# dist1ll/pomcpp

Hardware: AMD Instinct MI355X
Metric: env_steps_per_sec (higher is better)
Workload: dtype int32

## Files before the change

pomcpp_amd/csrc/pom_copy.h:

```cpp
#ifndef POM_COPY_H_
#define POM_COPY_H_

#include <hip/hip_runtime.h>

#include <cstdint>

#include "pom_batch.h"
#include "pom_kernels.h"
#include "pom_packed.h"

struct CopyParams {
    const int64_t* src;
    int64_t first, count, n, n_pad;
    int64_t tile0;
    int32_t flags;
    uint32_t* state;
    uint32_t* snap;
    uint32_t* agent_mem;
    uint32_t* episode;
    uint32_t* terminal;
    uint32_t* out_state;
    uint32_t* out_agent_mem;
    uint32_t* out_episode;
    uint32_t* out_terminal;
// ... 29 lines not shown
        } else {
            const uint32_t* st = p.state + (s >> 4) * POM_TILE_DWORDS;
            for (int k = lane; k < POM_COL_ITEMS; k += 64) pom_col_copy_item(tile, ec, st, (int)(s & 15), k);
        }
        if (p.agent_mem && lane < 8) {
            const int64_t half = (int64_t)(lane >> 2) * 4 * p.n_pad, a = lane & 3;
            p.out_agent_mem[half + e * 4 + a] = from_snap ? 0u : p.agent_mem[half + s * 4 + a];
        }
        if (!from_snap) {
            if (lane == 0) p.out_episode[e] = p.episode[s];
            if (p.terminal)
                for (int k = lane; k < POM_REC_DWORDS; k += 64) p.out_terminal[e * POM_REC_DWORDS + k] = p.terminal[s * POM_REC_DWORDS + k];
        }
    }
    __syncthreads();
    store_tile16_x4(p.out_state + t * POM_TILE_DWORDS, POM_TILE_ENVS, tile, lane);
}

template <bool SCATTER>
__global__ __launch_bounds__(64) void pom_copy_scatter_kernel(CopyParams p)
{
    const int lane = threadIdx.x;
    const int64_t t = p.tile0 + blockIdx.x;
    const bool from_snap = (p.flags & POM_COPY_FROM_SNAPSHOT) != 0;
    if (SCATTER) {
        const uint4* g = reinterpret_cast<const uint4*>(p.out_state + t * POM_TILE_DWORDS);
        uint4* d = reinterpret_cast<uint4*>(p.state + t * POM_TILE_DWORDS);
#pragma unroll
        for (int k = lane; k < POM_TILE_DWORDS / 4; k += 64) d[k] = g[k];
    }
    for (int ec = 0; ec < POM_TILE_ENVS; ec++) {
// ... 22 lines not shown
```

pomcpp_amd/csrc/pom_kernels.h:

```cpp
#ifndef POM_KERNELS_H_
#define POM_KERNELS_H_

#include <hip/hip_ext.h>
#include <hip/hip_runtime.h>

#include <climits>
#include <cstdint>

#include "pom_batch.h"
#include "pom_boardgen_body.h"
#include "pom_packed.h"
#include "pom_policy_body.h"
#include "pom_step_body.h"

enum {
    ROW_BOARD = POM_REC_BOARD,
    ROW_BOMBS = POM_REC_BOMBS,
    ROW_FLAMES = POM_REC_FLAMES,
    ROW_BDEST = POM_REC_DWORDS,
    ROW_STACK = POM_REC_DWORDS + 5,
    ROW_CLAIMS = POM_REC_DWORDS + 5,
    LDS_ROWS = POM_REC_DWORDS + 36
};
static_assert(POM_REC_DWORDS % 2 == 0, "the one-lane shapes move the record in groups of 1 or 2 rows");
// ... 63 lines not shown
#pragma unroll
        for (int k = 0; k < (31 + G - 1) / G; k++)
            if (G * k + G - 1 < 31 || sub() + G * k < 31) cm[sub() + G * k] = 0u;
    }
    __device__ void claim(int c)
    {
        __hip_atomic_fetch_add(reinterpret_cast<uint32_t*>(claim_map() + (c & ~3)), 1u << (8 * (c & 3)), __ATOMIC_RELAXED, __HIP_MEMORY_SCOPE_WORKGROUP);
    }
    __device__ int claims(int c) const { return claim_map()[c]; }
    __device__ void set_cell(int c, int v) { if (owner()) put_cell(c, v); }
    __device__ void set_bomb(int s, int v) { if (owner()) put_bomb(s, v); }
    __device__ void set_flame(int s, int v) { if (owner()) put_flame(s, v); }
    __device__ void set_bdest(int i, int v) { if (owner()) put_bdest(i, v); }
    __device__ void set_frame(int d, int v) { if (owner()) t[(ROW_STACK + d) * EPW] = (uint32_t)v; }
};

struct StepParams {
    uint32_t* state;
    const uint32_t* snap;
    const int32_t* moves;
    int64_t* wave_counters;
    int64_t n, n_pad, env_offset;
    uint64_t seed;
    uint32_t tick0;
    const uint32_t* tick_base;
    int32_t dist, ticks, mode, auto_reset, max_steps;
    int64_t block0, block_end;
    uint32_t* terminal;
    uint32_t* agent_mem;
    uint32_t* episode;
// ... 84 lines not shown
    }
}
template <int EPW>
__device__ __forceinline__ void store_tile(uint32_t* col, int64_t np, const uint32_t* tile, int sub, int el)
{
    constexpr int GR = 64 / EPW;
    uint32_t* g = col + (int64_t)sub * np;
    const int64_t stride = (int64_t)GR * np;
    const uint32_t* l = tile + sub * EPW + el;
#pragma unroll 8
    for (int r0 = 0; r0 < POM_REC_DWORDS; r0 += GR) {
        *g = l[r0 * EPW];
        g += stride;
    }
}
template <int ROWS = POM_REC_DWORDS, int AUX = 0>
__device__ __forceinline__ void load_tile16_x4(const uint32_t* base, int64_t np, uint32_t* tile, int lane)
{
    static_assert(ROWS <= POM_REC_DWORDS, "inside the record");
    const uint32_t* g = base + (int64_t)(lane >> 2) * np + 4 * (lane & 3);
    const int64_t stride = 16 * np;
#pragma unroll
    for (int r0 = 0; r0 + 16 <= ROWS; r0 += 16) {
        __builtin_amdgcn_global_load_lds((const __attribute__((address_space(1))) void*)g,
                                         (__attribute__((address_space(3))) void*)(tile + r0 * 16), 16, 0, AUX);
        g += stride;
    }
    if (ROWS % 16 != 0 && (lane >> 2) < ROWS % 16)
        __builtin_amdgcn_global_load_lds((const __attribute__((address_space(1))) void*)g,
                                         (__attribute__((address_space(3))) void*)(tile + (ROWS / 16) * 16 * 16), 16, 0, AUX);
}
template <bool NT = false>
__device__ __forceinline__ void store_tile16_x4(uint32_t* base, int64_t np, const uint32_t* tile, int lane)
{
    constexpr int ROWS = POM_REC_DWORDS;
    uint4* g = reinterpret_cast<uint4*>(base + (int64_t)(lane >> 2) * np + 4 * (lane & 3));
    const int64_t stride = 4 * np;
    const uint4* l = reinterpret_cast<const uint4*>(tile) + lane;
    typedef uint32_t pom_u32x4 __attribute__((ext_vector_type(4)));
#pragma unroll
    for (int r0 = 0; r0 + 16 <= ROWS; r0 += 16) {
        if (NT) {
            const uint4 v = l[r0 * 4];
            __builtin_nontemporal_store(pom_u32x4{v.x, v.y, v.z, v.w}, reinterpret_cast<pom_u32x4*>(g));
        } else *g = l[r0 * 4];
        g += stride;
    }
    if (ROWS % 16 != 0 && (lane >> 2) < ROWS % 16) {
        if (NT) {
            const uint4 v = l[(ROWS / 16) * 16 * 4];
            __builtin_nontemporal_store(pom_u32x4{v.x, v.y, v.z, v.w}, reinterpret_cast<pom_u32x4*>(g));
        } else *g = l[(ROWS / 16) * 16 * 4];
    }
}
template <int EPW, int ROWS = POM_REC_DWORDS>
__device__ __forceinline__ void restart_column(uint32_t* tile, int el, const uint32_t* src, int lane)
{
    const uint32_t v0 = src[lane];
    const uint32_t v1 = lane + 64 < ROWS ? src[lane + 64] : 0u;
    if (lane < POM_REC_BOARD_DWORDS) {
        uint8_t* cells = reinterpret_cast<uint8_t*>(tile);
#pragma unroll
        for (int j = 0; j < 4; j++) cells[tile_cell_byte<EPW>(el, 4 * lane + j)] = (uint8_t)(v0 >> (8 * j));
    } else tile[lane * EPW + el] = v0;
    if (lane + 64 < ROWS) tile[(lane + 64) * EPW + el] = v1;
}
template <int EPW>
__device__ __forceinline__ void column_to_record(const uint32_t* tile, int el, uint32_t* dst, int lane)
{
    if (lane < POM_REC_BOARD_DWORDS) {
        const uint8_t* cells = reinterpret_cast<const uint8_t*>(tile);
        uint32_t v = 0;
#pragma unroll
        for (int j = 0; j < 4; j++) v |= (uint32_t)cells[tile_cell_byte<EPW>(el, 4 * lane + j)] << (8 * j);
        dst[lane] = v;
    } else dst[lane] = tile[lane * EPW + el];
    if (lane + 64 < POM_REC_DWORDS) dst[lane + 64] = tile[(lane + 64) * EPW + el];
}

__device__ __forceinline__ void lane_from_tile(PomLane& L, int& time_step, uint32_t& status, const uint32_t* t, int epw)
// ... 562 lines not shown
__device__ __forceinline__ uint32_t pom_chain_xcd()
{
    uint32_t x;
    asm volatile("s_getreg_b32 %0, hwreg(HW_REG_XCC_ID)" : "=s"(x));
    return x & 0xFu;
}
__device__ __forceinline__ bool pom_chain_enter(unsigned long long* word, uint32_t chain_xcd, uint32_t chain_seq0, uint32_t tape_len, uint64_t wait_limit,
                                                uint32_t* err, int lane, PomChainVisit& v)
{
    const uint32_t xcd = chain_xcd + 1u;
#if defined(POM_CHAIN_DIAG)
    v.t0 = (long long)__builtin_readcyclecounter();
    v.rt0 = (long long)wall_clock64();
#endif
    unsigned long long w = 0;
    if (lane == 0) w = __hip_atomic_fetch_add(word, 1ull << POM_CHAIN_TICKET_SHIFT, __ATOMIC_RELAXED, __HIP_MEMORY_SCOPE_AGENT);
    w = ((unsigned long long)(uint32_t)__builtin_amdgcn_readfirstlane((int)(w >> 32)) << 32) | (uint32_t)__builtin_amdgcn_readfirstlane((int)(uint32_t)w);
    const uint32_t visit = (uint32_t)(w >> POM_CHAIN_TICKET_SHIFT);
    v.dist = (int32_t)pom_chain_visit_distance(visit, chain_seq0);
#if defined(POM_CHAIN_DIAG)
    v.t1 = (long long)__builtin_readcyclecounter();
#endif
    int polls = 0;
    bool timed_out = false;
    if (!((uint32_t)w & POM_CHAIN_POISON) && (int32_t)pom_chain_visit_distance((uint32_t)w & POM_CHAIN_COUNT_MASK, visit) < 0) {
        const uint64_t t_wait0 = wall_clock64();
        for (;;) {
            __builtin_amdgcn_s_sleep(1);
            w = __hip_atomic_load(word, __ATOMIC_RELAXED, __HIP_MEMORY_SCOPE_AGENT);
            w = ((unsigned long long)(uint32_t)__builtin_amdgcn_readfirstlane((int)(w >> 32)) << 32) | (uint32_t)__builtin_amdgcn_readfirstlane((int)(uint32_t)w);
            polls++;
            if (((uint32_t)w & POM_CHAIN_POISON) || (int32_t)pom_chain_visit_distance((uint32_t)w & POM_CHAIN_COUNT_MASK, visit) >= 0) break;
            if (wall_clock64() - t_wait0 >= wait_limit) {
                timed_out = true;
                break;
            }
        }
    }
    (void)polls;
    const uint32_t was_on = (uint32_t)(w >> 32) & 0xFu;
    const bool poisoned = ((uint32_t)w & POM_CHAIN_POISON) != 0;
    const bool wrong_xcd = was_on != 0u && was_on != xcd;
    const bool off_tape = tape_len != 0u && (uint32_t)v.dist >= tape_len;
    if (poisoned || timed_out || wrong_xcd || off_tape) {
        if (lane == 0 && !poisoned) {
            __hip_atomic_fetch_or(word, (unsigned long long)POM_CHAIN_POISON, __ATOMIC_RELAXED, __HIP_MEMORY_SCOPE_AGENT);
            __hip_atomic_fetch_or(err, (uint32_t)(timed_out ? POM_CHAIN_E_TIMEOUT : wrong_xcd ? POM_CHAIN_E_XCD : POM_CHAIN_E_TAPE), __ATOMIC_RELAXED,
                                  __HIP_MEMORY_SCOPE_AGENT);
        }
        return false;
    }
#if defined(POM_CHAIN_DIAG)
    v.t2 = (long long)__builtin_readcyclecounter();
    v.polls = polls;
    v.visit = visit;
#endif
    v.done = 1ull + ((unsigned long long)(xcd - was_on) << 32);
    return true;
}
__device__ __forceinline__ void pom_chain_leave(unsigned long long* word, int lane, const PomChainVisit& v)
{
    asm volatile("s_waitcnt vmcnt(0)" ::: "memory");
    if (lane == 0) __hip_atomic_fetch_add(word, v.done, __ATOMIC_RELAXED, __HIP_MEMORY_SCOPE_AGENT);
}

__device__ __forceinline__ int64_t pom_xcd_tile_order(int64_t b, int64_t nb)
{
    const int64_t q = nb / 8, r = nb % 8, x = b % 8;
    return (x < r ? x * (q + 1) : r * (q + 1) + (x - r) * q) + b / 8;
}

template <bool CHAIN>
__device__ __forceinline__ uint32_t pom_load_shared(const uint32_t* ptr)
{
    return CHAIN ? __hip_atomic_load(ptr, __ATOMIC_RELAXED, __HIP_MEMORY_SCOPE_AGENT) : *ptr;
}

template <int EPW, int G, bool FRESH, bool POLICY = false, bool ATEND = false, bool SINGLE = false, bool CHAIN = false, bool OBS = false>
// ... 6 lines not shown
    static_assert(!POLICY || G == 4, "the policy runs one agent per lane of the quad");
    static_assert(!ATEND || G == 4, "the end-of-tick reset is built for the quad shape only");
    constexpr int OBS_ROWS = (obs_stage_vecs(OBS_PASS_ENVS_FUSED) * 16 + EPW * 4 - 1) / (EPW * 4);
    constexpr int OVERLAY = POLICY ? 44 : OBS ? OBS_ROWS : 0;
    constexpr int ROWS = POM_REC_DWORDS + OVERLAY > LDS_ROWS ? POM_REC_DWORDS + OVERLAY : LDS_ROWS;
    static_assert(ROWS >= LDS_ROWS, "the tick's scratch rows fit under the overlay");
    __shared__ __attribute__((aligned(16))) uint32_t tiles_[POM_WPB][ROWS * EPW];
    uint32_t* const tile = tiles_[POM_WPB == 1 ? 0 : threadIdx.x >> 6];
    uint8_t* const danger = reinterpret_cast<uint8_t*>(tile + POM_REC_DWORDS * EPW);
    uint32_t* const sets = tile + (POM_REC_DWORDS + 32) * EPW;
    const int lane = threadIdx.x & 63;
    int64_t tile_local;
    uint32_t chain_xcd = 0;
    if (CHAIN) {
        chain_xcd = pom_chain_xcd();
        const int64_t q = gridDim.x / 8;
        int64_t k_in_xcd = (int64_t)(blockIdx.x / 8) + p.chain_rot;
        if (k_in_xcd >= q) k_in_xcd -= q;
        tile_local = (int64_t)chain_xcd * q + k_in_xcd;
        if (chain_xcd >= 8u) {
            if (lane == 0) __hip_atomic_fetch_or(p.chain_err, (uint32_t)POM_CHAIN_E_XCD, __ATOMIC_RELAXED, __HIP_MEMORY_SCOPE_AGENT);
            return;
        }
        if (POM_WPB == 1 && p.block0 + tile_local >= p.block_end) return;
    } else {
#if defined(POM_NO_XCD_REMAP)
    tile_local = blockIdx.x;
#else
    {
        const int64_t b = blockIdx.x, nb = gridDim.x, q = nb / 8, r = nb % 8, x = b % 8;
        tile_local = (x < r ? x * (q + 1) : r * (q + 1) + (x - r) * q) + b / 8;
    }
#endif
    }
    if (POM_WPB > 1) {
        tile_local = tile_local * POM_WPB + (threadIdx.x >> 6);
        if (p.block0 + tile_local >= p.block_end) return;
    }
    const int64_t tile_id = p.block0 + tile_local;
    const int64_t np = p.n_pad;
    const bool env_mode = p.mode == POM_MODE_ENV;
    const int el = lane % EPW, sub = lane / EPW;
    const int64_t e_d = tile_id * EPW + el;
    uint32_t* col_d = p.state + pom_rec_col(e_d);
    const int ec = G == 1 ? el : lane >> 2;
    const int member = G == 1 ? 0 : lane & 3;
    const int64_t e = tile_id * EPW + ec;
    const bool owner = G == 1 ? sub == 0 : member == 0;
    const bool runs = G == 1 ? sub == 0 : true;
    const bool valid = runs && e < p.n;
    const uint32_t env_key = (uint32_t)(p.env_offset + e);
    uint32_t* t = tile + ec;

#if defined(POM_DIAG)
    const long long t_begin = (long long)clock64();
#endif
    long long c_steps = 0, c_episodes = 0, c_resets = 0, c_ub = 0;

    uint32_t tick0 = CHAIN ? p.tick0 : p.tick0 + *p.tick_base;
    PomChainVisit cv;
    if (CHAIN) {
        unsigned long long* const word = p.tile_seq + tile_id * POM_CHAIN_WORD_STRIDE;
        if (!pom_chain_enter(word, chain_xcd, p.chain_seq0, p.tape_len, p.chain_wait_limit, p.chain_err, lane, cv)) return;
        tick0 += (uint32_t)cv.dist;
        load_tile16_x4<POM_REC_DWORDS, 16>(p.state + tile_id * POM_TILE_DWORDS, POM_TILE_ENVS, tile, lane);
    } else if (EPW == 16) load_tile16_x4(p.state + tile_id * POM_TILE_DWORDS, POM_TILE_ENVS, tile, lane);
    else load_tile<EPW>(col_d, POM_TILE_ENVS, tile, sub);
    uint32_t m0 = 0, m1 = 0;
    if (POLICY) {
        m0 = pom_load_shared<CHAIN>(p.agent_mem + tile_id * 64 + lane);
        m1 = pom_load_shared<CHAIN>(p.agent_mem + 4 * np + tile_id * 64 + lane);
    }
    uint64_t draw0 = 0;
    int4 moves0 = make_int4(0, 0, 0, 0);
    constexpr bool TAKES_MOVES = SINGLE || G == 1;
    if (!POLICY) {
        if (TAKES_MOVES && p.moves) {
            if (valid) moves0 = reinterpret_cast<const int4*>(p.moves)[(CHAIN ? (int64_t)cv.dist * p.n : (int64_t)0) + e];
        } else {
            if (G == 4 && !SINGLE) {
            } else if (G == 4) draw0 = pom_rng_draw_half(p.seed, env_key, tick0, member >> 1);
            else draw0 = pom_rng_draw(p.seed, env_key, tick0);
        }
    }
    asm volatile("s_waitcnt vmcnt(0)" ::: "memory");
    PomLane L;
    int time_step = 0;
    uint32_t status = 0;
    lane_from_tile(L, time_step, status, t, EPW);
    bool restarted = false;

    LdsEnv<EPW, G> acc(tile, ec, member);
    PomStepper<LdsEnv<EPW, G>> stepper(acc, L);
#if defined(POM_TRUNC)
    L.trunc = p.trunc;
#endif
#if defined(POM_DIAG)
    for (int k = 0; k < POM_PH_N; k++) L.t_acc[k] = 0;
    L.t_last = t_begin;
    POM_STAMP(L, POM_PH_LOAD);
#endif

    const int n_ticks = SINGLE ? 1 : p.ticks;
    for (int tk = 0; tk < n_ticks; tk++) {
        if (ATEND) {
        } else if (FRESH) {
            const bool reload = valid && env_mode && p.auto_reset == POM_RESET_AT_START && (status & POM_ST_DONE);
            uint64_t todo = __ballot(reload && owner);
            while (todo) {
                const int src = __builtin_amdgcn_readfirstlane(__ffsll((unsigned long long)todo) - 1);
                todo &= todo - 1;
                const int ec_u = G == 1 ? src : src >> 2;
                uint32_t ep = 0;
                if (lane == src) {
                    ep = pom_load_shared<CHAIN>(p.episode + e) + 1u;
                    p.episode[e] = ep;
                }
                ep = (uint32_t)__builtin_amdgcn_readfirstlane(__shfl((int)ep, src));
                const uint32_t key = pom_board_key(p.board_seed, (uint32_t)(p.env_offset + tile_id * EPW + ec_u), ep);
                pom_boardgen_wave<EPW, POM_REC_DWORDS>(tile, ec_u, (uint32_t)__builtin_amdgcn_readfirstlane((int)key), lane);
            }
            asm volatile("" ::: "memory");
            if (reload) lane_from_tile(L, time_step, status, t, EPW);
            restarted = reload;
            c_resets += __popcll(__ballot(reload && owner));
        } else {
            const bool reload = valid && env_mode && p.auto_reset == POM_RESET_AT_START && (status & POM_ST_DONE);
            uint64_t todo = __ballot(reload && owner);
            if (todo) {
                c_resets += __popcll(todo);
                int lane_now = lane;
                if (!SINGLE) asm volatile("" : "+v"(lane_now));
                do {
                    const int src = __builtin_amdgcn_readfirstlane(__ffsll((unsigned long long)todo) - 1);
                    todo &= todo - 1;
                    const int ec_u = G == 1 ? src : src >> 2;
                    restart_column<EPW>(tile, ec_u, p.snap + (tile_id * EPW + ec_u) * POM_REC_DWORDS, lane_now);
                } while (todo);
                asm volatile("" ::: "memory");
                if (reload) lane_from_tile(L, time_step, status, t, EPW);
            }
            restarted = reload;
        }
        const bool active = valid && !(env_mode && (status & POM_ST_DONE));
        bool newly_done = false, new_ub = false;
        int mv_own = POM_MOVE_IDLE;
        if (POLICY) {
            if (tk > 0) {
                m0 = p.agent_mem[tile_id * 64 + lane];
                m1 = p.agent_mem[4 * np + tile_id * 64 + lane];
            }
            if (restarted) m0 = m1 = 0;
            restarted = false;
            PolicyStore st{tile, t, danger + ec, sets + ec, member};
#if defined(POM_TRUNC)
            st.trunc = p.trunc;
            if (active) {
                if (p.trunc > -4) pom_policy_prepare_clear(st);
                if (p.trunc > -3) pom_policy_prepare_fill(st, PomPolicyEnv{{L.a0[0], L.a0[1], L.a0[2], L.a0[3]}, {acc.ag1(0), acc.ag1(1), acc.ag1(2), acc.ag1(3)}, L.bIdx, L.bCnt});
                if (p.trunc > -2) pom_policy_prepare_safe(st);
// ... 14 lines not shown
                long long pt_last = 0, pt_acc[POM_PP_N];
                mv_own = pom_policy_wave(st, E, member, m0, m1, actor, (int)((((r >> (16 * (member & 1))) & 0xFFFFu) * 5u) >> 16), sets, lane, pt_last, pt_acc);
#else
                mv_own = pom_policy_wave(st, E, member, m0, m1, actor, (int)((((r >> (16 * (member & 1))) & 0xFFFFu) * 5u) >> 16), sets, lane);
#endif
            }
            p.agent_mem[tile_id * 64 + lane] = m0;
            p.agent_mem[4 * np + tile_id * 64 + lane] = m1;
        }
        if (active) {
            uint32_t mvp;
            if (G == 4) {
                int mine;
                if (POLICY) {
                    mine = mv_own;
                } else if (TAKES_MOVES && p.moves) {
                    const int lo = (member & 1) ? moves0.y : moves0.x, hi = (member & 1) ? moves0.w : moves0.z;
                    mine = (member & 2) ? hi : lo;
                } else {
                    const uint32_t r = SINGLE ? (uint32_t)draw0 : pom_rng_draw_half(p.seed, env_key, tick0 + (uint32_t)tk, member >> 1);
                    mine = pom_rng_pick((r >> (16 * (member & 1))) & 0xFFFFu, p.dist);
                }
                mvp = stepper.pack_moves_quad(mine);
            } else {
                int mv[4];
                if (p.moves) {
                    mv[0] = moves0.x; mv[1] = moves0.y; mv[2] = moves0.z; mv[3] = moves0.w;
                } else {
                    const uint64_t r = tk == 0 ? draw0 : pom_rng_draw(p.seed, env_key, tick0 + (uint32_t)tk);
#pragma unroll
                    for (int i = 0; i < 4; i++) mv[i] = pom_rng_pick((uint32_t)(r >> (16 * i)) & 0xFFFFu, p.dist);
                }
                mvp = stepper.pack_moves(mv);
            }
            L.ub = 0;
            status &= ~(uint32_t)POM_ST_RESTARTED;
            POM_STAMP(L, POM_PH_RESTART);
#if defined(POM_TRUNC)
            if (p.trunc <= 0) {
            } else
#endif
            if (POLICY) {
                uint32_t* t2 = tile;
                asm volatile("" : "+v"(t2));
                LdsEnv<EPW, G> acc2(t2, ec, member);
                PomStepper<LdsEnv<EPW, G>> stepper2(acc2, L);
                stepper2.step_packed(mvp);
            } else {
                stepper.step_packed(mvp);
            }
            new_ub = L.ub != 0;
            L.ub |= (t[(POM_REC_AGENTS + 5) * EPW] >> 24) | ((t[(POM_REC_AGENTS + 7) * EPW] >> 24) << 8);
            if (env_mode) {
                time_step = (int)t[POM_REC_TIMESTEP * EPW] + 1;
                if (owner) t[POM_REC_TIMESTEP * EPW] = (uint32_t)time_step;
                status = pom_env_epilogue(L, time_step, p.max_steps, status);
                newly_done = (status & POM_ST_DONE) != 0;
            }
        }
        c_steps += __popcll(__ballot(active && owner));
        c_episodes += __popcll(__ballot(newly_done && owner));
        c_ub += __popcll(__ballot(new_ub && owner));
        if (ATEND) {
            uint64_t todo = __ballot(newly_done && owner);
            if (todo) {
                c_resets += __popcll(todo);
                if (newly_done && owner) {
#pragma unroll
                    for (int k = 0; k < 8; k++) t[(POM_REC_AGENTS + k) * EPW] = pom_lane_agent_word(L, status, k, t[(POM_REC_AGENTS + k) * EPW]);
                }
                asm volatile("" ::: "memory");
                int lane_end = lane;
                asm volatile("" : "+v"(lane_end));
                do {
                    const int src = __builtin_amdgcn_readfirstlane(__ffsll((unsigned long long)todo) - 1);
                    todo &= todo - 1;
                    const int ec_u = G == 1 ? src : src >> 2;
                    const int64_t e_u = tile_id * EPW + ec_u;
                    uint32_t* tr = p.terminal + e_u * POM_REC_DWORDS;
                    column_to_record<EPW>(tile, ec_u, tr, lane_end);
                    if (FRESH) {
                        uint32_t ep = 0;
                        if (lane == src) {
                            ep = pom_load_shared<CHAIN>(p.episode + e_u) + 1u;
                            p.episode[e_u] = ep;
                        }
                        ep = (uint32_t)__builtin_amdgcn_readfirstlane(__shfl((int)ep, src));
                        const uint32_t key = pom_board_key(p.board_seed, (uint32_t)(p.env_offset + e_u), ep);
                        pom_boardgen_wave<EPW, POM_REC_DWORDS>(tile, ec_u, (uint32_t)__builtin_amdgcn_readfirstlane((int)key), lane_end);
                    } else {
                        restart_column<EPW>(tile, ec_u, p.snap + e_u * POM_REC_DWORDS, lane_end);
                    }
                } while (todo);
                asm volatile("" ::: "memory");
                if (newly_done && runs) {
                    lane_from_tile(L, time_step, status, t, EPW);
                    status |= POM_ST_RESTARTED;
                    if (POLICY) {
                        int lane_here = lane;
                        asm volatile("" : "+v"(lane_here));
                        p.agent_mem[tile_id * 64 + lane_here] = 0u;
                        p.agent_mem[4 * np + tile_id * 64 + lane_here] = 0u;
                    }
                }
            }
        }
        POM_STAMP(L, POM_PH_EPILOGUE);
    }

    if (owner) {
#pragma unroll
        for (int k = 0; k < 8; k++) t[(POM_REC_AGENTS + k) * EPW] = pom_lane_agent_word(L, status, k, (k & 1) ? t[(POM_REC_AGENTS + k) * EPW] : 0u);
    }
    if (EPW == 16) {
        int lane_late = lane;
        asm volatile("" : "+v"(lane_late));
        store_tile16_x4<CHAIN>(p.state + tile_id * POM_TILE_DWORDS, POM_TILE_ENVS, tile, lane_late);
    } else {
        store_tile<EPW>(col_d, POM_TILE_ENVS, tile, sub, el);
    }
    if (OBS) {
        asm volatile("s_waitcnt lgkmcnt(0)" ::: "memory");
        ObserveParams op;
        op.state = nullptr;
        op.n = p.n;
        op.n_pad = p.n_pad;
        op.block0 = 0;
        op.planes = p.obs_planes;
        op.agent_attrs = p.obs_agent_attrs;
        op.env_attrs = p.obs_env_attrs;
        op.dtype = p.obs_dtype;
        op.per_agent = p.obs_per_agent;
// ... 18 lines not shown
    asm volatile("s_waitcnt vmcnt(0)" ::: "memory");
    POM_STAMP(L, POM_PH_STORE);
    if (p.diag) {
        long long inside = 0;
        for (int k = POM_PH_X_SCAN; k <= POM_PH_X_SHORT; k++) inside += L.t_acc[k];
        long long best = inside;
        for (int o = 32; o > 0; o >>= 1) {
            const long long w = __shfl_xor(best, o);
            best = w > best ? w : best;
        }
        const uint64_t who = __ballot(inside == best);
        if (lane == __ffsll((unsigned long long)who) - 1)
            for (int k = 0; k < POM_PH_N; k++) p.diag[tile_id * POM_PH_N + k] += L.t_acc[k];
    }
#endif
    if (lane == 0) {
        unsigned long long* wc = reinterpret_cast<unsigned long long*>(p.wave_counters + tile_id * POM_CNT_N);
        __hip_atomic_fetch_add(&wc[POM_CNT_STEPS], (unsigned long long)c_steps, __ATOMIC_RELAXED, __HIP_MEMORY_SCOPE_AGENT);
        if (c_episodes) __hip_atomic_fetch_add(&wc[POM_CNT_EPISODES], (unsigned long long)c_episodes, __ATOMIC_RELAXED, __HIP_MEMORY_SCOPE_AGENT);
        if (c_resets) __hip_atomic_fetch_add(&wc[POM_CNT_RESETS], (unsigned long long)c_resets, __ATOMIC_RELAXED, __HIP_MEMORY_SCOPE_AGENT);
        if (c_ub) __hip_atomic_fetch_add(&wc[POM_CNT_UB_TICKS], (unsigned long long)c_ub, __ATOMIC_RELAXED, __HIP_MEMORY_SCOPE_AGENT);
    }
}

struct LitmusParams {
    uint32_t* data;
    unsigned long long* tile_seq;
    uint32_t* err;
    unsigned long long* out;
    int64_t tiles;
    uint32_t chain_seq0;
    uint64_t wait_limit;
};
__global__ __launch_bounds__(64) void pom_chain_litmus_kernel(LitmusParams p)
{
    __shared__ __attribute__((aligned(16))) uint32_t tile[POM_REC_DWORDS * 16];
    const int lane = threadIdx.x;
    const uint32_t xcd = pom_chain_xcd();
    if (xcd >= 8u) return;
    const int64_t tile_id = (int64_t)xcd * (gridDim.x / 8) + blockIdx.x / 8;
    if (tile_id >= p.tiles) return;
    unsigned long long* const word = p.tile_seq + tile_id * POM_CHAIN_WORD_STRIDE;
    PomChainVisit cv;
    if (!pom_chain_enter(word, xcd, p.chain_seq0, 0u, p.wait_limit, p.err, lane, cv)) return;
    load_tile16_x4<POM_REC_DWORDS, 16>(p.data + tile_id * POM_TILE_DWORDS, POM_TILE_ENVS, tile, lane);
    asm volatile("s_waitcnt vmcnt(0)" ::: "memory");
    const uint32_t expect = p.chain_seq0 + (uint32_t)cv.dist;
    const uint32_t tag = (uint32_t)tile_id * 2654435761u;
    int bad = 0;
#pragma unroll 4
    for (int k = lane; k < POM_TILE_DWORDS; k += 64) {
        bad += tile[k] != (expect ^ (tag + (uint32_t)k));
        tile[k] = (expect + 1u) ^ (tag + (uint32_t)k);
    }
    for (int o = 32; o > 0; o >>= 1) bad += __shfl_xor(bad, o);
    asm volatile("s_waitcnt lgkmcnt(0)" ::: "memory");
    store_tile16_x4<true>(p.data + tile_id * POM_TILE_DWORDS, POM_TILE_ENVS, tile, lane);
    pom_chain_leave(word, lane, cv);
    if (lane == 0) {
        if (bad) {
            atomicAdd(p.out + 0, 1ull);
            atomicAdd(p.out + 1, (unsigned long long)bad);
        }
        atomicAdd(p.out + 2, 1ull);
    }
}

__global__ void pom_chain_probe_kernel(uint32_t* xcd_of_block)
{
    uint32_t x;
    asm volatile("s_getreg_b32 %0, hwreg(HW_REG_XCC_ID)" : "=s"(x));
    if (threadIdx.x == 0) xcd_of_block[blockIdx.x] = x & 0xFu;
// ... 38 lines not shown
};

__global__ __launch_bounds__(64) void pom_policy_kernel(PolicyParams p)
{
    __shared__ __attribute__((aligned(16))) uint32_t tile[POL_LOAD_ROWS * 16];
    __shared__ uint8_t danger[128 * 16];
    __shared__ uint32_t sets[12 * 16];
    const int lane = threadIdx.x;
    const int64_t np = p.n_pad;
    const int64_t tile_local = pom_xcd_tile_order(blockIdx.x, gridDim.x);
    const int64_t tile_id = p.block0 + tile_local;
    const bool env_mode = p.mode == POM_MODE_ENV;
#if defined(POM_DIAG)
    long long t_last = (long long)clock64(), t_acc[POM_PP_N] = {0, 0, 0, 0, 0, 0, 0};
#endif
    load_tile16_x4<POL_LOAD_ROWS>(p.state + tile_id * POM_TILE_DWORDS, POM_TILE_ENVS, tile, lane);
    const int ec = lane >> 2, id = lane & 3;
    const int64_t e = tile_id * 16 + ec;
    const int64_t slot = e * 4 + id;
    uint32_t m0 = p.agent_mem[slot], m1 = p.agent_mem[4 * np + slot];
    asm volatile("s_waitcnt vmcnt(0)" ::: "memory");
    const bool restart = e < p.n && env_mode && p.auto_reset == POM_RESET_AT_START && ((pom_rec_meta2(tile + ec, 16) >> 8) & POM_ST_DONE);
    if (restart) m0 = m1 = 0;
    {
        uint64_t todo = __ballot(restart && id == 0);
        while (todo) {
            const int src = __builtin_amdgcn_readfirstlane(__ffsll((unsigned long long)todo) - 1);
            todo &= todo - 1;
            const int ec_u = src >> 2;
            if (p.fresh) {
                const uint32_t ep = p.episode[tile_id * 16 + ec_u] + 1u;
// ... 49 lines not shown
        }
        t_acc[k] = v;
    }
    if (lane == 0 && p.diag)
        for (int k = 0; k < POM_PP_N; k++) p.diag[tile_id * POM_PP_N + k] += t_acc[k];
#endif
}

__global__ __launch_bounds__(64) void pom_observe_kernel(ObserveParams p)
{
    __shared__ __attribute__((aligned(16))) uint32_t tile[POM_REC_DWORDS * 16];
    __shared__ uint4 stage[obs_stage_vecs(OBS_PASS_ENVS_ALONE)];
    const int lane = threadIdx.x;
    const int64_t tile_local = pom_xcd_tile_order(blockIdx.x, gridDim.x);
    const int64_t tile_id = p.block0 + tile_local;
    load_tile16_x4(p.state + tile_id * POM_TILE_DWORDS, POM_TILE_ENVS, tile, lane);
    __builtin_amdgcn_s_waitcnt(0x0F70);
    asm volatile("" ::: "memory");
    pom_observe_tile<OBS_PASS_ENVS_ALONE>(p, tile, stage, tile_id, lane);
}

__global__ __launch_bounds__(64) void pom_generate_kernel(uint32_t* state, uint32_t* snap, uint32_t* episode, int64_t n, int64_t np,
                                                          int64_t env_offset, uint64_t board_seed)
{
    __shared__ __attribute__((aligned(16))) uint32_t tile[POM_REC_DWORDS * 16];
    const int lane = threadIdx.x;
    const int64_t tile_id = blockIdx.x;
    if (tile_id * 16 + 16 > n) {
        for (int k = lane; k < POM_REC_DWORDS * 4; k += 64) reinterpret_cast<uint4*>(tile)[k] = make_uint4(0, 0, 0, 0);
        __syncthreads();
    }
    for (int ec = 0; ec < 16 && tile_id * 16 + ec < n; ec++)
        pom_boardgen_wave<16, POM_REC_DWORDS>(tile, ec, pom_board_key(board_seed, (uint32_t)(env_offset + tile_id * 16 + ec), 0u), lane);
    if (tile_id * 16 + lane < n && lane < 16) episode[tile_id * 16 + lane] = 0u;
    __syncthreads();
    store_tile16_x4(state + tile_id * POM_TILE_DWORDS, POM_TILE_ENVS, tile, lane);
    for (int ec = 0; ec < 16; ec++) {
        column_to_record<16>(tile, ec, snap + (tile_id * 16 + ec) * POM_REC_DWORDS, lane);
    }
}

#include "pom_boundary.h"

__global__ __launch_bounds__(1024) void pom_reduce_counters_kernel(const int64_t* __restrict__ wc, int64_t n_waves, int64_t* out)
{
    __shared__ long long part[POM_CNT_N][16];
    long long acc[POM_CNT_N] = {0, 0, 0, 0};
    for (int64_t w = threadIdx.x; w < n_waves; w += blockDim.x) {
        const longlong2 lo = *reinterpret_cast<const longlong2*>(wc + w * POM_CNT_N);
        const longlong2 hi = *reinterpret_cast<const longlong2*>(wc + w * POM_CNT_N + 2);
        acc[0] += lo.x; acc[1] += lo.y; acc[2] += hi.x; acc[3] += hi.y;
// ... 16 lines not shown
```

Before: 8.982 billion.

## Move step-kernel bookkeeping to scalar masks and immediate-offset tile copies

Many lane-level predicates (owner, valid, reload, newly_done) become precomputed 64-bit exec masks with inverse-ballot, so the per-tick ballots go away. Tile load and store now use scalar base pointers with constant immediate offsets instead of per-lane 64-bit stride arithmetic. The snapshot restarts are batched two records at a time so their fetches overlap, and the four counter atomics are merged into one lane-parallel atomic. Counters become 32-bit in single-tick mode. These changes aim to cut VALU and SGPR/VGPR overhead in the hot step kernel, but they rely on inline-asm register hints and assume the tile layout matches the fixed offsets.

```diff
diff --git a/pomcpp_amd/csrc/pom_copy.h b/pomcpp_amd/csrc/pom_copy.h
--- a/pomcpp_amd/csrc/pom_copy.h
+++ b/pomcpp_amd/csrc/pom_copy.h
@@ -67,7 +67,7 @@
         }
     }
     __syncthreads();
-    store_tile16_x4(p.out_state + t * POM_TILE_DWORDS, POM_TILE_ENVS, tile, lane);
+    store_tile16_x4(p.out_state + t * POM_TILE_DWORDS, tile, lane);
 }
 
 template <bool SCATTER>
diff --git a/pomcpp_amd/csrc/pom_kernels.h b/pomcpp_amd/csrc/pom_kernels.h
--- a/pomcpp_amd/csrc/pom_kernels.h
+++ b/pomcpp_amd/csrc/pom_kernels.h
@@ -6,6 +6,8 @@
 
 #include <climits>
 #include <cstdint>
+#include <type_traits>
+#include <utility>
 
 #include "pom_batch.h"
 #include "pom_boardgen_body.h"
@@ -101,6 +103,32 @@
     __device__ void set_bdest(int i, int v) { if (owner()) put_bdest(i, v); }
     __device__ void set_frame(int d, int v) { if (owner()) t[(ROW_STACK + d) * EPW] = (uint32_t)v; }
 };
+
+__device__ __forceinline__ uint64_t pom_mask_nz(uint32_t v) { return __builtin_amdgcn_uicmp(v, 0u, 33 ); }
+__device__ __forceinline__ bool pom_lanes(uint64_t mask) { return __builtin_amdgcn_inverse_ballot_w64(mask); }
+__device__ __forceinline__ int pom_scalar_late(int uniform)
+{
+    asm volatile("" : "+s"(uniform));
+    return uniform;
+}
+__device__ __forceinline__ bool pom_scalar_less(int64_t a, int64_t b)
+{
+    return pom_scalar_late((int)(((uint64_t)a - (uint64_t)b) >> 32)) < 0;
+}
+template <class T>
+__device__ __forceinline__ T* pom_scalar_base(T* uniform)
+{
+    asm volatile("" : "+s"(uniform));
+    return uniform;
+}
+__device__ __forceinline__ uint64_t pom_first_lanes(int count) { return count >= 64 ? ~0ull : (1ull << count) - 1ull; }
+template <class T>
+__device__ __forceinline__ T* pom_one_lane_address(T* uniform)
+{
+    uint32_t zero = 0u;
+    asm volatile("" : "+v"(zero));
+    return reinterpret_cast<T*>(reinterpret_cast<char*>(uniform) + zero);
+}
 
 struct StepParams {
     uint32_t* state;
@@ -215,56 +243,89 @@
         g += stride;
     }
 }
+typedef const __attribute__((address_space(1))) char* pom_gptr;
+typedef __attribute__((address_space(3))) char* pom_lptr;
+template <int ROWS, int AUX, int GRP>
+__device__ __forceinline__ void load_tile16_group(const uint32_t* base, uint32_t* tile, int lane)
+{
+    constexpr int G0 = GRP / 4 * 4;
+    const pom_gptr g = (pom_gptr)(G0 == 0 ? base : pom_scalar_base(base + G0 * 256)) + (uint32_t)lane * 16u;
+    const pom_lptr l = (pom_lptr)(tile + G0 * 256);
+    if ((GRP + 1) * 16 <= ROWS || (lane >> 2) < ROWS % 16)
+        __builtin_amdgcn_global_load_lds(g, l, 16, (GRP - G0) * 1024, AUX);
+}
+template <int ROWS, int AUX, int... GRP>
+__device__ __forceinline__ void load_tile16_groups(const uint32_t* base, uint32_t* tile, int lane, std::integer_sequence<int, GRP...>)
+{
+    (load_tile16_group<ROWS, AUX, GRP>(base, tile, lane), ...);
+}
 template <int ROWS = POM_REC_DWORDS, int AUX = 0>
-__device__ __forceinline__ void load_tile16_x4(const uint32_t* base, int64_t np, uint32_t* tile, int lane)
+__device__ __forceinline__ void load_tile16_x4(const uint32_t* base, uint32_t* tile, int lane)
 {
     static_assert(ROWS <= POM_REC_DWORDS, "inside the record");
-    const uint32_t* g = base + (int64_t)(lane >> 2) * np + 4 * (lane & 3);
-    const int64_t stride = 16 * np;
-#pragma unroll
-    for (int r0 = 0; r0 + 16 <= ROWS; r0 += 16) {
-        __builtin_amdgcn_global_load_lds((const __attribute__((address_space(1))) void*)g,
-                                         (__attribute__((address_space(3))) void*)(tile + r0 * 16), 16, 0, AUX);
-        g += stride;
-    }
-    if (ROWS % 16 != 0 && (lane >> 2) < ROWS % 16)
-        __builtin_amdgcn_global_load_lds((const __attribute__((address_space(1))) void*)g,
-                                         (__attribute__((address_space(3))) void*)(tile + (ROWS / 16) * 16 * 16), 16, 0, AUX);
+    load_tile16_groups<ROWS, AUX>(base, tile, lane, std::make_integer_sequence<int, (ROWS + 15) / 16>{});
 }
 template <bool NT = false>
-__device__ __forceinline__ void store_tile16_x4(uint32_t* base, int64_t np, const uint32_t* tile, int lane)
+__device__ __forceinline__ void store_tile16_x4(uint32_t* base, const uint32_t* tile, int lane)
 {
     constexpr int ROWS = POM_REC_DWORDS;
-    uint4* g = reinterpret_cast<uint4*>(base + (int64_t)(lane >> 2) * np + 4 * (lane & 3));
-    const int64_t stride = 4 * np;
+    static_assert(ROWS % 16 == 0 && ROWS * 64 <= 2 * 2048 + 1024, "whole row groups, all within the immediate's reach of the tile's middle");
+    typedef uint32_t pom_u32x4 __attribute__((ext_vector_type(4)));
+    const uint32_t off = (uint32_t)lane * 16u;
+    typedef __attribute__((address_space(1))) char* gchar;
+    typedef __attribute__((address_space(1))) pom_u32x4* gvec;
+    const gchar g = (gchar)pom_scalar_base(reinterpret_cast<char*>(base) + 2048) + off;
     const uint4* l = reinterpret_cast<const uint4*>(tile) + lane;
-    typedef uint32_t pom_u32x4 __attribute__((ext_vector_type(4)));
-#pragma unroll
-    for (int r0 = 0; r0 + 16 <= ROWS; r0 += 16) {
-        if (NT) {
-            const uint4 v = l[r0 * 4];
-            __builtin_nontemporal_store(pom_u32x4{v.x, v.y, v.z, v.w}, reinterpret_cast<pom_u32x4*>(g));
-        } else *g = l[r0 * 4];
-        g += stride;
-    }
-    if (ROWS % 16 != 0 && (lane >> 2) < ROWS % 16) {
-        if (NT) {
-            const uint4 v = l[(ROWS / 16) * 16 * 4];
-            __builtin_nontemporal_store(pom_u32x4{v.x, v.y, v.z, v.w}, reinterpret_cast<pom_u32x4*>(g));
-        } else *g = l[(ROWS / 16) * 16 * 4];
-    }
+#pragma unroll
+    for (int r0 = 0; r0 < ROWS; r0 += 16) {
+        const gvec d = (gvec)(g + (r0 * 64 - 2048));
+        const uint4 v = l[r0 * 4];
+        if (NT) __builtin_nontemporal_store(pom_u32x4{v.x, v.y, v.z, v.w}, d);
+        else *d = pom_u32x4{v.x, v.y, v.z, v.w};
+    }
+}
+template <int ROWS = POM_REC_DWORDS>
+__device__ __forceinline__ void restart_fetch(const uint32_t* src, int lane, uint32_t& v0, uint32_t& v1)
+{
+    typedef const __attribute__((address_space(1))) uint32_t* gword;
+    const pom_gptr s = (pom_gptr)pom_scalar_base(reinterpret_cast<const char*>(src)) + (uint32_t)lane * 4u;
+    v0 = *(gword)s;
+    v1 = lane + 64 < ROWS ? *(gword)(s + 256) : 0u;
 }
 template <int EPW, int ROWS = POM_REC_DWORDS>
-__device__ __forceinline__ void restart_column(uint32_t* tile, int el, const uint32_t* src, int lane)
-{
-    const uint32_t v0 = src[lane];
-    const uint32_t v1 = lane + 64 < ROWS ? src[lane + 64] : 0u;
+__device__ __forceinline__ void restart_scatter(uint32_t* tile, int el, int lane, uint32_t v0, uint32_t v1)
+{
     if (lane < POM_REC_BOARD_DWORDS) {
         uint8_t* cells = reinterpret_cast<uint8_t*>(tile);
 #pragma unroll
         for (int j = 0; j < 4; j++) cells[tile_cell_byte<EPW>(el, 4 * lane + j)] = (uint8_t)(v0 >> (8 * j));
     } else tile[lane * EPW + el] = v0;
     if (lane + 64 < ROWS) tile[(lane + 64) * EPW + el] = v1;
+}
+template <int EPW, int ROWS = POM_REC_DWORDS>
+__device__ __forceinline__ void restart_column(uint32_t* tile, int el, const uint32_t* src, int lane)
+{
+    uint32_t v0, v1;
+    restart_fetch<ROWS>(src, lane, v0, v1);
+    restart_scatter<EPW, ROWS>(tile, el, lane, v0, v1);
+}
+template <int EPW, int G, int ROWS = POM_REC_DWORDS>
+__device__ __forceinline__ void restart_columns(uint32_t* tile, uint64_t todo, const uint32_t* snap_tile, int lane)
+{
+    do {
+        const int ea = pom_scalar_late(__builtin_ctzll(todo) / G);
+        todo &= todo - 1;
+        uint32_t a0, a1;
+        restart_fetch<ROWS>(snap_tile + ea * POM_REC_DWORDS, lane, a0, a1);
+        if (todo) {
+            const int eb = pom_scalar_late(__builtin_ctzll(todo) / G);
+            todo &= todo - 1;
+            uint32_t b0, b1;
+            restart_fetch<ROWS>(snap_tile + eb * POM_REC_DWORDS, lane, b0, b1);
+            restart_scatter<EPW, ROWS>(tile, ea, lane, a0, a1);
+            restart_scatter<EPW, ROWS>(tile, eb, lane, b0, b1);
+        } else restart_scatter<EPW, ROWS>(tile, ea, lane, a0, a1);
+    } while (todo);
 }
 template <int EPW>
 __device__ __forceinline__ void column_to_record(const uint32_t* tile, int el, uint32_t* dst, int lane)
@@ -857,7 +918,7 @@
     v.rt0 = (long long)wall_clock64();
 #endif
     unsigned long long w = 0;
-    if (lane == 0) w = __hip_atomic_fetch_add(word, 1ull << POM_CHAIN_TICKET_SHIFT, __ATOMIC_RELAXED, __HIP_MEMORY_SCOPE_AGENT);
+    if (pom_lanes(1ull)) w = __hip_atomic_fetch_add(pom_one_lane_address(word), 1ull << POM_CHAIN_TICKET_SHIFT, __ATOMIC_RELAXED, __HIP_MEMORY_SCOPE_AGENT);
     w = ((unsigned long long)(uint32_t)__builtin_amdgcn_readfirstlane((int)(w >> 32)) << 32) | (uint32_t)__builtin_amdgcn_readfirstlane((int)(uint32_t)w);
     const uint32_t visit = (uint32_t)(w >> POM_CHAIN_TICKET_SHIFT);
     v.dist = (int32_t)pom_chain_visit_distance(visit, chain_seq0);
@@ -887,9 +948,9 @@
     const bool off_tape = tape_len != 0u && (uint32_t)v.dist >= tape_len;
     if (poisoned || timed_out || wrong_xcd || off_tape) {
         if (lane == 0 && !poisoned) {
-            __hip_atomic_fetch_or(word, (unsigned long long)POM_CHAIN_POISON, __ATOMIC_RELAXED, __HIP_MEMORY_SCOPE_AGENT);
-            __hip_atomic_fetch_or(err, (uint32_t)(timed_out ? POM_CHAIN_E_TIMEOUT : wrong_xcd ? POM_CHAIN_E_XCD : POM_CHAIN_E_TAPE), __ATOMIC_RELAXED,
-                                  __HIP_MEMORY_SCOPE_AGENT);
+            __hip_atomic_fetch_or(pom_one_lane_address(word), (unsigned long long)POM_CHAIN_POISON, __ATOMIC_RELAXED, __HIP_MEMORY_SCOPE_AGENT);
+            __hip_atomic_fetch_or(pom_one_lane_address(err), (uint32_t)(timed_out ? POM_CHAIN_E_TIMEOUT : wrong_xcd ? POM_CHAIN_E_XCD : POM_CHAIN_E_TAPE),
+                                  __ATOMIC_RELAXED, __HIP_MEMORY_SCOPE_AGENT);
         }
         return false;
     }
@@ -904,7 +965,7 @@
 __device__ __forceinline__ void pom_chain_leave(unsigned long long* word, int lane, const PomChainVisit& v)
 {
     asm volatile("s_waitcnt vmcnt(0)" ::: "memory");
-    if (lane == 0) __hip_atomic_fetch_add(word, v.done, __ATOMIC_RELAXED, __HIP_MEMORY_SCOPE_AGENT);
+    if (pom_lanes(1ull)) __hip_atomic_fetch_add(pom_one_lane_address(word), v.done, __ATOMIC_RELAXED, __HIP_MEMORY_SCOPE_AGENT);
 }
 
 __device__ __forceinline__ int64_t pom_xcd_tile_order(int64_t b, int64_t nb)
@@ -941,15 +1002,15 @@
     uint32_t chain_xcd = 0;
     if (CHAIN) {
         chain_xcd = pom_chain_xcd();
-        const int64_t q = gridDim.x / 8;
-        int64_t k_in_xcd = (int64_t)(blockIdx.x / 8) + p.chain_rot;
+        const uint32_t q = gridDim.x / 8;
+        uint32_t k_in_xcd = blockIdx.x / 8 + p.chain_rot;
         if (k_in_xcd >= q) k_in_xcd -= q;
         tile_local = (int64_t)chain_xcd * q + k_in_xcd;
         if (chain_xcd >= 8u) {
-            if (lane == 0) __hip_atomic_fetch_or(p.chain_err, (uint32_t)POM_CHAIN_E_XCD, __ATOMIC_RELAXED, __HIP_MEMORY_SCOPE_AGENT);
+            if (pom_lanes(1ull)) __hip_atomic_fetch_or(pom_one_lane_address(p.chain_err), (uint32_t)POM_CHAIN_E_XCD, __ATOMIC_RELAXED, __HIP_MEMORY_SCOPE_AGENT);
             return;
         }
-        if (POM_WPB == 1 && p.block0 + tile_local >= p.block_end) return;
+        if (POM_WPB == 1 && !pom_scalar_less(p.block0 + tile_local, p.block_end)) return;
     } else {
 #if defined(POM_NO_XCD_REMAP)
     tile_local = blockIdx.x;
@@ -967,22 +1028,28 @@
     const int64_t tile_id = p.block0 + tile_local;
     const int64_t np = p.n_pad;
     const bool env_mode = p.mode == POM_MODE_ENV;
+    int mode_held = p.mode;
+    const bool restarts = env_mode && p.auto_reset == POM_RESET_AT_START;
     const int el = lane % EPW, sub = lane / EPW;
     const int64_t e_d = tile_id * EPW + el;
     uint32_t* col_d = p.state + pom_rec_col(e_d);
     const int ec = G == 1 ? el : lane >> 2;
     const int member = G == 1 ? 0 : lane & 3;
     const int64_t e = tile_id * EPW + ec;
-    const bool owner = G == 1 ? sub == 0 : member == 0;
+    constexpr uint64_t OWNERS = G == 4 ? 0x1111111111111111ull : EPW == 64 ? ~0ull : (1ull << (EPW & 63)) - 1ull;
+    const bool owner = pom_lanes(OWNERS);
     const bool runs = G == 1 ? sub == 0 : true;
-    const bool valid = runs && e < p.n;
+    const int64_t envs_left = p.n - tile_id * EPW;
+    const int valid_envs = !pom_scalar_less(envs_left, EPW) ? EPW : pom_scalar_less(envs_left, 0) ? 0 : (int)envs_left;
+    const uint64_t valid_m = pom_first_lanes(G * valid_envs);
     const uint32_t env_key = (uint32_t)(p.env_offset + e);
     uint32_t* t = tile + ec;
 
 #if defined(POM_DIAG)
     const long long t_begin = (long long)clock64();
 #endif
-    long long c_steps = 0, c_episodes = 0, c_resets = 0, c_ub = 0;
+    typedef typename std::conditional<SINGLE, uint32_t, uint64_t>::type count_t;
+    count_t c_steps = 0, c_episodes = 0, c_resets = 0, c_ub = 0;
 
     uint32_t tick0 = CHAIN ? p.tick0 : p.tick0 + *p.tick_base;
     PomChainVisit cv;
@@ -990,31 +1057,35 @@
         unsigned long long* const word = p.tile_seq + tile_id * POM_CHAIN_WORD_STRIDE;
         if (!pom_chain_enter(word, chain_xcd, p.chain_seq0, p.tape_len, p.chain_wait_limit, p.chain_err, lane, cv)) return;
         tick0 += (uint32_t)cv.dist;
-        load_tile16_x4<POM_REC_DWORDS, 16>(p.state + tile_id * POM_TILE_DWORDS, POM_TILE_ENVS, tile, lane);
-    } else if (EPW == 16) load_tile16_x4(p.state + tile_id * POM_TILE_DWORDS, POM_TILE_ENVS, tile, lane);
+        load_tile16_x4<POM_REC_DWORDS, 16>(p.state + tile_id * POM_TILE_DWORDS, tile, lane);
+    } else if (EPW == 16) load_tile16_x4(p.state + tile_id * POM_TILE_DWORDS, tile, lane);
     else load_tile<EPW>(col_d, POM_TILE_ENVS, tile, sub);
     uint32_t m0 = 0, m1 = 0;
     if (POLICY) {
         m0 = pom_load_shared<CHAIN>(p.agent_mem + tile_id * 64 + lane);
         m1 = pom_load_shared<CHAIN>(p.agent_mem + 4 * np + tile_id * 64 + lane);
     }
+    constexpr bool TAKES_MOVES = SINGLE || G == 1;
     uint64_t draw0 = 0;
     int4 moves0 = make_int4(0, 0, 0, 0);
-    constexpr bool TAKES_MOVES = SINGLE || G == 1;
+    uint32_t mine0 = 0;
     if (!POLICY) {
         if (TAKES_MOVES && p.moves) {
-            if (valid) moves0 = reinterpret_cast<const int4*>(p.moves)[(CHAIN ? (int64_t)cv.dist * p.n : (int64_t)0) + e];
+            const int32_t* const mv = p.moves + ((CHAIN ? (int64_t)cv.dist * p.n : (int64_t)0) + tile_id * EPW) * 4;
+            if (G == 4) {
+                if (pom_lanes(valid_m)) mine0 = (uint32_t)*reinterpret_cast<const int32_t*>(reinterpret_cast<const char*>(mv) + (uint32_t)lane * 4u);
+            } else if (pom_lanes(valid_m)) moves0 = *reinterpret_cast<const int4*>(reinterpret_cast<const char*>(mv) + (uint32_t)ec * 16u);
         } else {
             if (G == 4 && !SINGLE) {
-            } else if (G == 4) draw0 = pom_rng_draw_half(p.seed, env_key, tick0, member >> 1);
+            } else if (G == 4)
+                mine0 = (uint32_t)pom_rng_pick((pom_rng_draw_half(p.seed, env_key, tick0, member >> 1) >> (16 * (member & 1))) & 0xFFFFu, p.dist);
             else draw0 = pom_rng_draw(p.seed, env_key, tick0);
         }
     }
     asm volatile("s_waitcnt vmcnt(0)" ::: "memory");
     PomLane L;
     int time_step = 0;
-    uint32_t status = 0;
-    lane_from_tile(L, time_step, status, t, EPW);
+    uint32_t status = t[(POM_REC_AGENTS + 3) * EPW] >> 24;
     bool restarted = false;
 
     LdsEnv<EPW, G> acc(tile, ec, member);
@@ -1031,11 +1102,14 @@
     const int n_ticks = SINGLE ? 1 : p.ticks;
     for (int tk = 0; tk < n_ticks; tk++) {
         if (ATEND) {
+            if (tk == 0) lane_from_tile(L, time_step, status, t, EPW);
         } else if (FRESH) {
-            const bool reload = valid && env_mode && p.auto_reset == POM_RESET_AT_START && (status & POM_ST_DONE);
-            uint64_t todo = __ballot(reload && owner);
+            const uint64_t reload_m = restarts ? pom_mask_nz(status & POM_ST_DONE) & valid_m : 0ull;
+            const bool reload = pom_lanes(reload_m);
+            uint64_t todo = reload_m & OWNERS;
+            c_resets += __popcll(todo);
             while (todo) {
-                const int src = __builtin_amdgcn_readfirstlane(__ffsll((unsigned long long)todo) - 1);
+                const int src = __builtin_ctzll(todo);
                 todo &= todo - 1;
                 const int ec_u = G == 1 ? src : src >> 2;
                 uint32_t ep = 0;
@@ -1043,34 +1117,30 @@
                     ep = pom_load_shared<CHAIN>(p.episode + e) + 1u;
                     p.episode[e] = ep;
                 }
-                ep = (uint32_t)__builtin_amdgcn_readfirstlane(__shfl((int)ep, src));
+                ep = (uint32_t)__builtin_amdgcn_readlane((int)ep, src);
                 const uint32_t key = pom_board_key(p.board_seed, (uint32_t)(p.env_offset + tile_id * EPW + ec_u), ep);
                 pom_boardgen_wave<EPW, POM_REC_DWORDS>(tile, ec_u, (uint32_t)__builtin_amdgcn_readfirstlane((int)key), lane);
             }
             asm volatile("" ::: "memory");
-            if (reload) lane_from_tile(L, time_step, status, t, EPW);
+            if (tk == 0 || reload) lane_from_tile(L, time_step, status, t, EPW);
             restarted = reload;
-            c_resets += __popcll(__ballot(reload && owner));
         } else {
-            const bool reload = valid && env_mode && p.auto_reset == POM_RESET_AT_START && (status & POM_ST_DONE);
-            uint64_t todo = __ballot(reload && owner);
+            const uint64_t reload_m = restarts ? pom_mask_nz(status & POM_ST_DONE) & valid_m : 0ull;
+            const bool reload = pom_lanes(reload_m);
+            const uint64_t todo = reload_m & OWNERS;
             if (todo) {
                 c_resets += __popcll(todo);
                 int lane_now = lane;
                 if (!SINGLE) asm volatile("" : "+v"(lane_now));
-                do {
-                    const int src = __builtin_amdgcn_readfirstlane(__ffsll((unsigned long long)todo) - 1);
-                    todo &= todo - 1;
-                    const int ec_u = G == 1 ? src : src >> 2;
-                    restart_column<EPW>(tile, ec_u, p.snap + (tile_id * EPW + ec_u) * POM_REC_DWORDS, lane_now);
-                } while (todo);
+                restart_columns<EPW, G>(tile, todo, p.snap + tile_id * (EPW * POM_REC_DWORDS), lane_now);
                 asm volatile("" ::: "memory");
-                if (reload) lane_from_tile(L, time_step, status, t, EPW);
-            }
+            }
+            if (tk == 0 || reload) lane_from_tile(L, time_step, status, t, EPW);
             restarted = reload;
         }
-        const bool active = valid && !(env_mode && (status & POM_ST_DONE));
-        bool newly_done = false, new_ub = false;
+        const uint64_t active_m = valid_m & ~(env_mode ? pom_mask_nz(status & POM_ST_DONE) : 0ull);
+        const bool active = pom_lanes(active_m);
+        uint32_t tick_ub = 0;
         int mv_own = POM_MOVE_IDLE;
         if (POLICY) {
             if (tk > 0) {
@@ -1115,12 +1185,11 @@
                 int mine;
                 if (POLICY) {
                     mine = mv_own;
-                } else if (TAKES_MOVES && p.moves) {
-                    const int lo = (member & 1) ? moves0.y : moves0.x, hi = (member & 1) ? moves0.w : moves0.z;
-                    mine = (member & 2) ? hi : lo;
+                } else if (SINGLE) {
+                    mine = (int)mine0;
                 } else {
-                    const uint32_t r = SINGLE ? (uint32_t)draw0 : pom_rng_draw_half(p.seed, env_key, tick0 + (uint32_t)tk, member >> 1);
-                    mine = pom_rng_pick((r >> (16 * (member & 1))) & 0xFFFFu, p.dist);
+                    const uint32_t r16 = (pom_rng_draw_half(p.seed, env_key, tick0 + (uint32_t)tk, member >> 1) >> (16 * (member & 1))) & 0xFFFFu;
+                    mine = pom_rng_pick(r16, p.dist);
                 }
                 mvp = stepper.pack_moves_quad(mine);
             } else {
@@ -1150,22 +1219,23 @@
             } else {
                 stepper.step_packed(mvp);
             }
-            new_ub = L.ub != 0;
+            tick_ub = L.ub;
             L.ub |= (t[(POM_REC_AGENTS + 5) * EPW] >> 24) | ((t[(POM_REC_AGENTS + 7) * EPW] >> 24) << 8);
-            if (env_mode) {
+            if (pom_scalar_late(mode_held) == POM_MODE_ENV) {
                 time_step = (int)t[POM_REC_TIMESTEP * EPW] + 1;
                 if (owner) t[POM_REC_TIMESTEP * EPW] = (uint32_t)time_step;
                 status = pom_env_epilogue(L, time_step, p.max_steps, status);
-                newly_done = (status & POM_ST_DONE) != 0;
-            }
-        }
-        c_steps += __popcll(__ballot(active && owner));
-        c_episodes += __popcll(__ballot(newly_done && owner));
-        c_ub += __popcll(__ballot(new_ub && owner));
+            }
+        }
+        const uint64_t newly_done_m = pom_scalar_late(mode_held) == POM_MODE_ENV ? pom_mask_nz(status & POM_ST_DONE) & active_m : 0ull;
+        c_steps += __popcll(active_m & OWNERS);
+        c_episodes += __popcll(newly_done_m & OWNERS);
+        c_ub += __popcll(pom_mask_nz(tick_ub) & OWNERS);
         if (ATEND) {
-            uint64_t todo = __ballot(newly_done && owner);
+            uint64_t todo = newly_done_m & OWNERS;
             if (todo) {
                 c_resets += __popcll(todo);
+                const bool newly_done = pom_lanes(newly_done_m);
                 if (newly_done && owner) {
 #pragma unroll
                     for (int k = 0; k < 8; k++) t[(POM_REC_AGENTS + k) * EPW] = pom_lane_agent_word(L, status, k, t[(POM_REC_AGENTS + k) * EPW]);
@@ -1173,9 +1243,10 @@
                 asm volatile("" ::: "memory");
                 int lane_end = lane;
                 asm volatile("" : "+v"(lane_end));
+                uint64_t out = todo;
                 do {
-                    const int src = __builtin_amdgcn_readfirstlane(__ffsll((unsigned long long)todo) - 1);
-                    todo &= todo - 1;
+                    const int src = __builtin_ctzll(out);
+                    out &= out - 1;
                     const int ec_u = G == 1 ? src : src >> 2;
                     const int64_t e_u = tile_id * EPW + ec_u;
                     uint32_t* tr = p.terminal + e_u * POM_REC_DWORDS;
@@ -1186,13 +1257,15 @@
                             ep = pom_load_shared<CHAIN>(p.episode + e_u) + 1u;
                             p.episode[e_u] = ep;
                         }
-                        ep = (uint32_t)__builtin_amdgcn_readfirstlane(__shfl((int)ep, src));
+                        ep = (uint32_t)__builtin_amdgcn_readlane((int)ep, src);
                         const uint32_t key = pom_board_key(p.board_seed, (uint32_t)(p.env_offset + e_u), ep);
                         pom_boardgen_wave<EPW, POM_REC_DWORDS>(tile, ec_u, (uint32_t)__builtin_amdgcn_readfirstlane((int)key), lane_end);
-                    } else {
-                        restart_column<EPW>(tile, ec_u, p.snap + e_u * POM_REC_DWORDS, lane_end);
                     }
-                } while (todo);
+                } while (out);
+                if (!FRESH) {
+                    asm volatile("" ::: "memory");
+                    restart_columns<EPW, G>(tile, todo, p.snap + tile_id * (EPW * POM_REC_DWORDS), lane_end);
+                }
                 asm volatile("" ::: "memory");
                 if (newly_done && runs) {
                     lane_from_tile(L, time_step, status, t, EPW);
@@ -1216,7 +1289,7 @@
     if (EPW == 16) {
         int lane_late = lane;
         asm volatile("" : "+v"(lane_late));
-        store_tile16_x4<CHAIN>(p.state + tile_id * POM_TILE_DWORDS, POM_TILE_ENVS, tile, lane_late);
+        store_tile16_x4<CHAIN>(p.state + tile_id * POM_TILE_DWORDS, tile, lane_late);
     } else {
         store_tile<EPW>(col_d, POM_TILE_ENVS, tile, sub, el);
     }
@@ -1265,12 +1338,22 @@
             for (int k = 0; k < POM_PH_N; k++) p.diag[tile_id * POM_PH_N + k] += L.t_acc[k];
     }
 #endif
-    if (lane == 0) {
-        unsigned long long* wc = reinterpret_cast<unsigned long long*>(p.wave_counters + tile_id * POM_CNT_N);
-        __hip_atomic_fetch_add(&wc[POM_CNT_STEPS], (unsigned long long)c_steps, __ATOMIC_RELAXED, __HIP_MEMORY_SCOPE_AGENT);
-        if (c_episodes) __hip_atomic_fetch_add(&wc[POM_CNT_EPISODES], (unsigned long long)c_episodes, __ATOMIC_RELAXED, __HIP_MEMORY_SCOPE_AGENT);
-        if (c_resets) __hip_atomic_fetch_add(&wc[POM_CNT_RESETS], (unsigned long long)c_resets, __ATOMIC_RELAXED, __HIP_MEMORY_SCOPE_AGENT);
-        if (c_ub) __hip_atomic_fetch_add(&wc[POM_CNT_UB_TICKS], (unsigned long long)c_ub, __ATOMIC_RELAXED, __HIP_MEMORY_SCOPE_AGENT);
+    {
+        static_assert(POM_CNT_STEPS == 0 && POM_CNT_EPISODES == 1 && POM_CNT_RESETS == 2 && POM_CNT_UB_TICKS == 3 && POM_CNT_N == 4, "lane k: counter k");
+        int lane_cnt = lane;
+        asm volatile("" : "+v"(lane_cnt));
+        unsigned long long* const wc = reinterpret_cast<unsigned long long*>(
+            reinterpret_cast<char*>(p.wave_counters + tile_id * POM_CNT_N) + (uint32_t)lane_cnt * 8u);
+        const count_t sums[4] = {c_steps, c_episodes, c_resets, c_ub};
+        uint32_t lo = (uint32_t)sums[0], hi = SINGLE ? 0u : (uint32_t)((uint64_t)sums[0] >> 32);
+        uint32_t who = sums[0] ? 1u : 0u;
+#pragma unroll
+        for (int k = 1; k < 4; k++) {
+            lo = pom_lanes(1ull << k) ? (uint32_t)sums[k] : lo;
+            if (!SINGLE) hi = pom_lanes(1ull << k) ? (uint32_t)((uint64_t)sums[k] >> 32) : hi;
+            who |= sums[k] ? 1u << k : 0u;
+        }
+        if (pom_lanes(who)) __hip_atomic_fetch_add(wc, ((unsigned long long)hi << 32) | lo, __ATOMIC_RELAXED, __HIP_MEMORY_SCOPE_AGENT);
     }
 }
 
@@ -1294,7 +1377,7 @@
     unsigned long long* const word = p.tile_seq + tile_id * POM_CHAIN_WORD_STRIDE;
     PomChainVisit cv;
     if (!pom_chain_enter(word, xcd, p.chain_seq0, 0u, p.wait_limit, p.err, lane, cv)) return;
-    load_tile16_x4<POM_REC_DWORDS, 16>(p.data + tile_id * POM_TILE_DWORDS, POM_TILE_ENVS, tile, lane);
+    load_tile16_x4<POM_REC_DWORDS, 16>(p.data + tile_id * POM_TILE_DWORDS, tile, lane);
     asm volatile("s_waitcnt vmcnt(0)" ::: "memory");
     const uint32_t expect = p.chain_seq0 + (uint32_t)cv.dist;
     const uint32_t tag = (uint32_t)tile_id * 2654435761u;
@@ -1306,7 +1389,7 @@
     }
     for (int o = 32; o > 0; o >>= 1) bad += __shfl_xor(bad, o);
     asm volatile("s_waitcnt lgkmcnt(0)" ::: "memory");
-    store_tile16_x4<true>(p.data + tile_id * POM_TILE_DWORDS, POM_TILE_ENVS, tile, lane);
+    store_tile16_x4<true>(p.data + tile_id * POM_TILE_DWORDS, tile, lane);
     pom_chain_leave(word, lane, cv);
     if (lane == 0) {
         if (bad) {
@@ -1375,7 +1458,7 @@
 #if defined(POM_DIAG)
     long long t_last = (long long)clock64(), t_acc[POM_PP_N] = {0, 0, 0, 0, 0, 0, 0};
 #endif
-    load_tile16_x4<POL_LOAD_ROWS>(p.state + tile_id * POM_TILE_DWORDS, POM_TILE_ENVS, tile, lane);
+    load_tile16_x4<POL_LOAD_ROWS>(p.state + tile_id * POM_TILE_DWORDS, tile, lane);
     const int ec = lane >> 2, id = lane & 3;
     const int64_t e = tile_id * 16 + ec;
     const int64_t slot = e * 4 + id;
@@ -1455,7 +1538,7 @@
     const int lane = threadIdx.x;
     const int64_t tile_local = pom_xcd_tile_order(blockIdx.x, gridDim.x);
     const int64_t tile_id = p.block0 + tile_local;
-    load_tile16_x4(p.state + tile_id * POM_TILE_DWORDS, POM_TILE_ENVS, tile, lane);
+    load_tile16_x4(p.state + tile_id * POM_TILE_DWORDS, tile, lane);
     __builtin_amdgcn_s_waitcnt(0x0F70);
     asm volatile("" ::: "memory");
     pom_observe_tile<OBS_PASS_ENVS_ALONE>(p, tile, stage, tile_id, lane);
@@ -1475,7 +1558,7 @@
         pom_boardgen_wave<16, POM_REC_DWORDS>(tile, ec, pom_board_key(board_seed, (uint32_t)(env_offset + tile_id * 16 + ec), 0u), lane);
     if (tile_id * 16 + lane < n && lane < 16) episode[tile_id * 16 + lane] = 0u;
     __syncthreads();
-    store_tile16_x4(state + tile_id * POM_TILE_DWORDS, POM_TILE_ENVS, tile, lane);
+    store_tile16_x4(state + tile_id * POM_TILE_DWORDS, tile, lane);
     for (int ec = 0; ec < 16; ec++) {
         column_to_record<16>(tile, ec, snap + (tile_id * 16 + ec) * POM_REC_DWORDS, lane);
     }
```

Measured after the change: 9.400 billion, median of 6. +4.6%, better.
